# lucasnewman/f5-tts-mlx

Measured on NVIDIA H100. Metric: mel-frames/sec, higher is better.
Workload: dtype bf16

## Files before the change

### f5_tts_mlx_b200/csrc/attention_sm90.cuh

```cuda
#pragma once
#include "ptx.cuh"

namespace f5 {

struct AttnParams {
  int B, N, H;
  const int* kv_len;
  __nv_bfloat16* out;
  int ldo;
  unsigned long long* prof;
  int out_fp8;
  float* scale_out;
};

struct AttnSmem {
  static constexpr int kQ = 0;
  static constexpr int kK = 16384;
  static constexpr int kV = kK + 2 * 16384;
  static constexpr int kBar = kV + 2 * 16384;
  static constexpr int kNumBars = 9;
  static constexpr int kTotal = kBar + kNumBars * 8 + 1024;
};

template <bool kOut8, bool kScaled = false>
__global__ void __launch_bounds__(384, 1)
attn_fwd_kernel(const __grid_constant__ CUtensorMap tma_qkv, const AttnParams p) {
  extern __shared__ uint8_t smem_raw[];
  uint8_t* smem = smem_raw + ((1024u - (smem_u32(smem_raw) & 1023u)) & 1023u);
  uint64_t* bars = reinterpret_cast<uint64_t*>(smem + AttnSmem::kBar);
  uint64_t* q_full = bars + 0;
  uint64_t* k_full = bars + 1;
  uint64_t* k_empty = bars + 3;
  uint64_t* v_full = bars + 5;
  uint64_t* v_empty = bars + 7;

  const int warp = threadIdx.x >> 5, lane = threadIdx.x & 31;
  const int q0 = blockIdx.x * 128;
  const int h = blockIdx.y;
  const int b = blockIdx.z;
  const int HD = p.H * 64;

  if (warp == 0 && F5_ELECT_LANE()) {
    tma_prefetch_desc(&tma_qkv);
    mbar_init(q_full, 1);
    for (int i = 0; i < 2; ++i) {
      mbar_init(&k_full[i], 1);
      mbar_init(&k_empty[i], 256);
      mbar_init(&v_full[i], 1);
      mbar_init(&v_empty[i], 256);
    }
    fence_mbar_init();
  }
  __syncthreads();
  pdl_wait();
  if (threadIdx.x == 128) prof_stamp_begin(p.prof);
  int kv_len = p.kv_len ? p.kv_len[b] : p.N;
  kv_len = min(max(kv_len, 1), p.N);
  const int num_kv = (kv_len + 127) >> 7;

  if (warp < 4) {
    if (warp == 0 && F5_ELECT_LANE()) {
      mbar_expect_tx(q_full, 16384);
      tma_load_3d(smem + AttnSmem::kQ, &tma_qkv, q_full, h * 64, q0, b);
      for (int j = 0; j < num_kv; ++j) {
        const int s = j & 1;
        const uint32_t ph = (j >> 1) & 1;
        mbar_wait(&k_empty[s], ph ^ 1);
        mbar_expect_tx(&k_full[s], 16384);
        tma_load_3d(smem + AttnSmem::kK + s * 16384, &tma_qkv, &k_full[s], HD + h * 64, j * 128, b);
        mbar_wait(&v_empty[s], ph ^ 1);
        mbar_expect_tx(&v_full[s], 16384);
        tma_load_3d(smem + AttnSmem::kV + s * 16384, &tma_qkv, &v_full[s], 2 * HD + h * 64, j * 128, b);
      }
    }
  } else {
    const int wg = (threadIdx.x >> 7) - 1;
    const int rw = ((threadIdx.x >> 5) & 3) * 16 + (lane >> 2);
    const uint32_t sQ = smem_u32(smem + AttnSmem::kQ) + wg * (64 * 128);
    constexpr float kLog2e = 1.4426950408889634f;
    float o[32];
#pragma unroll
    for (int i = 0; i < 32; ++i) o[i] = 0.f;
    float m_run[2] = {-INFINITY, -INFINITY}, l_run[2] = {0.f, 0.f};
    mbar_wait(q_full, 0);

    for (int j = 0; j < num_kv; ++j) {
      const int s = j & 1;
      const uint32_t ph = (j >> 1) & 1;
      float sv[64];
      mbar_wait(&k_full[s], ph);
      const uint32_t sK = smem_u32(smem + AttnSmem::kK + s * 16384);
      wgmma_fence();
#pragma unroll
      for (int k = 0; k < 4; ++k)
        wgmma_bf16_ss_n128(sv, gmma_desc_sw128(sQ + 32 * k, 16, 1024), gmma_desc_sw128(sK + 32 * k, 16, 1024), k != 0);
      wgmma_commit();
      wgmma_wait<0>();
      wgmma_reg_fence(sv);
      mbar_arrive(&k_empty[s]);

      const int kv0 = j * 128;
      if (kv0 + 128 > kv_len) {
#pragma unroll
        for (int i = 0; i < 64; ++i)
          if (kv0 + 8 * (i >> 2) + 2 * (lane & 3) + (i & 1) >= kv_len) sv[i] = -INFINITY;
      }
      float mx[2] = {m_run[0], m_run[1]};
#pragma unroll
      for (int i = 0; i < 64; ++i) mx[(i >> 1) & 1] = fmaxf(mx[(i >> 1) & 1], sv[i]);
#pragma unroll
      for (int r = 0; r < 2; ++r) {
        mx[r] = fmaxf(mx[r], __shfl_xor_sync(0xffffffffu, mx[r], 1));
        mx[r] = fmaxf(mx[r], __shfl_xor_sync(0xffffffffu, mx[r], 2));
      }
      float sc[2], mb[2];
#pragma unroll
      for (int r = 0; r < 2; ++r) {
        sc[r] = ex2_approx((m_run[r] - mx[r]) * kLog2e);
        m_run[r] = mx[r];
        mb[r] = mx[r] * kLog2e;
        l_run[r] *= sc[r];
      }
#pragma unroll
      for (int i = 0; i < 32; ++i) o[i] *= sc[(i >> 1) & 1];
      uint32_t pa[8][4];
#pragma unroll
      for (int kk = 0; kk < 8; ++kk) {
#pragma unroll
        for (int m = 0; m < 4; ++m) {
          const int i = 8 * kk + 2 * m, r = m & 1;
          const float e0 = ex2_approx(fmaf(sv[i], kLog2e, -mb[r]));
          const float e1 = ex2_approx(fmaf(sv[i + 1], kLog2e, -mb[r]));
          l_run[r] += e0 + e1;
          pa[kk][m] = pack_bf16x2(e0, e1);
        }
      }

      mbar_wait(&v_full[s], ph);
      const uint32_t sV = smem_u32(smem + AttnSmem::kV + s * 16384);
      wgmma_fence();
#pragma unroll
      for (int kk = 0; kk < 8; ++kk) wgmma_bf16_rs_n64_tb(o, pa[kk], gmma_desc_sw128(sV + kk * 2048, 16384, 1024));
      wgmma_commit();
      wgmma_wait<0>();
      wgmma_reg_fence(o);
      mbar_arrive(&v_empty[s]);
    }

    pdl_launch_dependents();
#pragma unroll
    for (int r = 0; r < 2; ++r) {
      l_run[r] += __shfl_xor_sync(0xffffffffu, l_run[r], 1);
      l_run[r] += __shfl_xor_sync(0xffffffffu, l_run[r], 2);
    }
    const float inv[2] = {1.f / l_run[0], 1.f / l_run[1]};
    float qs[2] = {1.f, 1.f}, qinv[2] = {1.f, 1.f};
    if constexpr (kScaled) {
#pragma unroll
      for (int r = 0; r < 2; ++r) {
        float amax = 0.f;
#pragma unroll
        for (int c = 0; c < 8; ++c)
          amax = fmax_nan(amax, fmax_nan(fabsf(o[4 * c + 2 * r] * inv[r]), fabsf(o[4 * c + 2 * r + 1] * inv[r])));
        amax = fmax_nan(amax, __shfl_xor_sync(0xffffffffu, amax, 1));
        amax = fmax_nan(amax, __shfl_xor_sync(0xffffffffu, amax, 2));
        qs[r] = e4m3_block_scale(amax, qinv[r]);
      }
    }
#pragma unroll
    for (int r = 0; r < 2; ++r) {
      const int n = q0 + wg * 64 + rw + 8 * r;
      if (n >= p.N) continue;
      const size_t row = (size_t)b * p.N + n;
      if (kScaled && (lane & 3) == 0) p.scale_out[(size_t)h * p.B * p.N + row] = qs[r];
#pragma unroll
      for (int c = 0; c < 8; ++c) {
        const int col = h * 64 + 8 * c + 2 * (lane & 3);
        float v0 = o[4 * c + 2 * r] * inv[r], v1 = o[4 * c + 2 * r + 1] * inv[r];
        if constexpr (kScaled) { v0 *= qinv[r]; v1 *= qinv[r]; }
        if constexpr (kOut8) {
          uint16_t w;
          asm("cvt.rn.satfinite.e4m3x2.f32 %0, %1, %2;" : "=h"(w) : "f"(v1), "f"(v0));
          *reinterpret_cast<uint16_t*>(reinterpret_cast<uint8_t*>(p.out) + row * p.ldo + col) = w;
        } else {
          *reinterpret_cast<uint32_t*>(p.out + row * p.ldo + col) = pack_bf16x2(v0, v1);
        }
      }
    }
  }

  __syncthreads();
  if (threadIdx.x == 0) prof_stamp_end(p.prof);
}

}
```

Baseline: 8148.

## Overlap QK and PV wgmma across iterations with warpgroup ping-pong scheduling

```diff
diff --git a/f5_tts_mlx_b200/csrc/attention_sm90.cuh b/f5_tts_mlx_b200/csrc/attention_sm90.cuh
--- a/f5_tts_mlx_b200/csrc/attention_sm90.cuh
+++ b/f5_tts_mlx_b200/csrc/attention_sm90.cuh
@@ -59,6 +59,7 @@
   const int num_kv = (kv_len + 127) >> 7;
 
   if (warp < 4) {
+    asm volatile("setmaxnreg.dec.sync.aligned.u32 24;\n");
     if (warp == 0 && F5_ELECT_LANE()) {
       mbar_expect_tx(q_full, 16384);
       tma_load_3d(smem + AttnSmem::kQ, &tma_qkv, q_full, h * 64, q0, b);
@@ -74,6 +75,7 @@
       }
     }
   } else {
+    asm volatile("setmaxnreg.inc.sync.aligned.u32 240;\n");
     const int wg = (threadIdx.x >> 7) - 1;
     const int rw = ((threadIdx.x >> 5) & 3) * 16 + (lane >> 2);
     const uint32_t sQ = smem_u32(smem + AttnSmem::kQ) + wg * (64 * 128);
@@ -82,23 +84,25 @@
 #pragma unroll
     for (int i = 0; i < 32; ++i) o[i] = 0.f;
     float m_run[2] = {-INFINITY, -INFINITY}, l_run[2] = {0.f, 0.f};
+    float sv[64];
+    uint32_t pa[8][4];
+    float sc[2];
     mbar_wait(q_full, 0);
 
-    for (int j = 0; j < num_kv; ++j) {
-      const int s = j & 1;
-      const uint32_t ph = (j >> 1) & 1;
-      float sv[64];
-      mbar_wait(&k_full[s], ph);
-      const uint32_t sK = smem_u32(smem + AttnSmem::kK + s * 16384);
-      wgmma_fence();
+    auto issue_s = [&](int j) {
+      const uint32_t sK = smem_u32(smem + AttnSmem::kK + (j & 1) * 16384);
 #pragma unroll
       for (int k = 0; k < 4; ++k)
         wgmma_bf16_ss_n128(sv, gmma_desc_sw128(sQ + 32 * k, 16, 1024), gmma_desc_sw128(sK + 32 * k, 16, 1024), k != 0);
       wgmma_commit();
-      wgmma_wait<0>();
-      wgmma_reg_fence(sv);
-      mbar_arrive(&k_empty[s]);
-
+    };
+    auto issue_pv = [&](int j) {
+      const uint32_t sV = smem_u32(smem + AttnSmem::kV + (j & 1) * 16384);
+#pragma unroll
+      for (int kk = 0; kk < 8; ++kk) wgmma_bf16_rs_n64_tb(o, pa[kk], gmma_desc_sw128(sV + kk * 2048, 16384, 1024));
+      wgmma_commit();
+    };
+    auto softmax = [&](int j) {
       const int kv0 = j * 128;
       if (kv0 + 128 > kv_len) {
 #pragma unroll
@@ -113,7 +117,7 @@
         mx[r] = fmaxf(mx[r], __shfl_xor_sync(0xffffffffu, mx[r], 1));
         mx[r] = fmaxf(mx[r], __shfl_xor_sync(0xffffffffu, mx[r], 2));
       }
-      float sc[2], mb[2];
+      float mb[2];
 #pragma unroll
       for (int r = 0; r < 2; ++r) {
         sc[r] = ex2_approx((m_run[r] - mx[r]) * kLog2e);
@@ -122,30 +126,66 @@
         l_run[r] *= sc[r];
       }
 #pragma unroll
-      for (int i = 0; i < 32; ++i) o[i] *= sc[(i >> 1) & 1];
-      uint32_t pa[8][4];
-#pragma unroll
       for (int kk = 0; kk < 8; ++kk) {
 #pragma unroll
         for (int m = 0; m < 4; ++m) {
           const int i = 8 * kk + 2 * m, r = m & 1;
-          const float e0 = ex2_approx(fmaf(sv[i], kLog2e, -mb[r]));
-          const float e1 = ex2_approx(fmaf(sv[i + 1], kLog2e, -mb[r]));
-          l_run[r] += e0 + e1;
-          pa[kk][m] = pack_bf16x2(e0, e1);
+          sv[i] = ex2_approx(fmaf(sv[i], kLog2e, -mb[r]));
+          sv[i + 1] = ex2_approx(fmaf(sv[i + 1], kLog2e, -mb[r]));
+          l_run[r] += sv[i] + sv[i + 1];
         }
       }
-
-      mbar_wait(&v_full[s], ph);
-      const uint32_t sV = smem_u32(smem + AttnSmem::kV + s * 16384);
+    };
+    auto rescale_and_pack = [&]() {
+#pragma unroll
+      for (int i = 0; i < 32; ++i) o[i] *= sc[(i >> 1) & 1];
+#pragma unroll
+      for (int kk = 0; kk < 8; ++kk)
+#pragma unroll
+        for (int m = 0; m < 4; ++m) pa[kk][m] = pack_bf16x2(sv[8 * kk + 2 * m], sv[8 * kk + 2 * m + 1]);
+    };
+
+    auto turn_wait = [&]() { asm volatile("bar.sync %0, 256;" ::"r"(1 + wg) : "memory"); };
+    auto turn_pass = [&](bool last) {
+      if (wg == 0 || !last) asm volatile("bar.arrive %0, 256;" ::"r"(2 - wg) : "memory");
+    };
+    if (wg == 1) asm volatile("bar.arrive 1, 256;" ::: "memory");
+    mbar_wait(&k_full[0], 0);
+    turn_wait();
+    wgmma_fence();
+    issue_s(0);
+    turn_pass(num_kv == 1);
+    wgmma_wait<0>();
+    wgmma_reg_fence(sv);
+    mbar_arrive(&k_empty[0]);
+    softmax(0);
+    mbar_wait(&v_full[0], 0);
+    rescale_and_pack();
+    for (int j = 0; j + 1 < num_kv; ++j) {
+      const int sn = (j + 1) & 1, s = j & 1;
+      const uint32_t phn = ((j + 1) >> 1) & 1;
+      mbar_wait(&k_full[sn], phn);
+      turn_wait();
       wgmma_fence();
-#pragma unroll
-      for (int kk = 0; kk < 8; ++kk) wgmma_bf16_rs_n64_tb(o, pa[kk], gmma_desc_sw128(sV + kk * 2048, 16384, 1024));
-      wgmma_commit();
+      issue_s(j + 1);
+      issue_pv(j);
+      turn_pass(j + 2 == num_kv);
+      wgmma_wait<1>();
+      wgmma_reg_fence(sv);
+      mbar_arrive(&k_empty[sn]);
+      softmax(j + 1);
+      mbar_wait(&v_full[sn], phn);
       wgmma_wait<0>();
       wgmma_reg_fence(o);
       mbar_arrive(&v_empty[s]);
-    }
+      rescale_and_pack();
+    }
+    const int jl = num_kv - 1;
+    wgmma_fence();
+    issue_pv(jl);
+    wgmma_wait<0>();
+    wgmma_reg_fence(o);
+    mbar_arrive(&v_empty[jl & 1]);
 
     pdl_launch_dependents();
 #pragma unroll
```

New measurement: 8255, median of 6. 1.01x the previous value.
